# KKKSQJ/DeepLearning

Measured on NVIDIA H100. Metric: images/sec (ResNet-50 training step), higher is better.
Workload: dtype bf16

## Files before the change

deeplearning_b200/csrc/abi_conv.cu:

```cuda
#include <string.h>
#include "../../include/b200cls.h"
#include "conv_gemm.cuh"
#include "conv1x1_stream.cuh"
#include "conv_tap64.cuh"
#include "host_utils.h"
#include "wgrad_gemm.cuh"

using namespace b200;

namespace {

constexpr uint32_t kFwdDescLbo = 16, kFwdDescSbo = 1024;
constexpr uint32_t kWgDescLbo = 8192, kWgDescSbo = 1024, kWgDescKstep = 2048;

struct Box3 {
  int b1, b2, b3;
};

Box3 choose_box(long long d1, long long d2, long long d3, int P) {
  Box3 best{P, 1, 1};
  double best_cost = -1;
  for (int b1 = 1; b1 <= P; b1 <<= 1) {
    for (int b2 = 1; b1 * b2 <= P; b2 <<= 1) {
      const int b3 = P / (b1 * b2);
      if (b1 > 256 || b2 > 256 || b3 > 256) continue;
      const double c1 = double((d1 + b1 - 1) / b1) * b1, c2 = double((d2 + b2 - 1) / b2) * b2,
                   c3 = double((d3 + b3 - 1) / b3) * b3;
      const double cost = c1 * c2 * c3;
      if (best_cost < 0 || cost < best_cost - 0.5 ||
          (cost < best_cost + 0.5 && (b1 > best.b1 || (b1 == best.b1 && b2 > best.b2)))) {
        best_cost = cost;
        best = Box3{b1, b2, b3};
      }
    }
  }
  return best;
}

inline int pad_of(int ksize) { return ksize == 2 ? 0 : ksize / 2; }
inline int out_dim(int in, int ksize, int stride) { return (in + 2 * pad_of(ksize) - ksize) / stride + 1; }

struct Dims3 {
  long long d1, d2, d3;
};
Dims3 out_dims(int B, int H, int W, int ksize, int stride) {
  if (ksize == 1 && stride == 1) return Dims3{static_cast<long long>(B) * H * W, 1, 1};
  return Dims3{out_dim(W, ksize, stride), out_dim(H, ksize, stride), B};
}

struct View {
  const void* base;
  uint64_t dims[4];
  uint64_t strides[4];
};

View make_view(const void* base, int B, int H, int W, int C, int s, int ph, int pw) {
  View v;
  v.base = static_cast<const char*>(base) + (static_cast<long long>(ph) * W + pw) * C * 2;
  v.dims[0] = C;
  v.dims[1] = (W - pw + s - 1) / s;
  v.dims[2] = (H - ph + s - 1) / s;
  v.dims[3] = B;
  v.strides[0] = 1;
  v.strides[1] = static_cast<uint64_t>(s) * C;
  v.strides[2] = static_cast<uint64_t>(s) * W * C;
  v.strides[3] = static_cast<uint64_t>(H) * W * C;
  return v;
}
View make_flat_view(const void* base, long long M, int C) {
  View v;
  v.base = base;
  v.dims[0] = C;
  v.dims[1] = M;
  v.dims[2] = 1;
  v.dims[3] = 1;
  v.strides[0] = 1;
  v.strides[1] = C;
  v.strides[2] = static_cast<uint64_t>(M) * C;
  v.strides[3] = static_cast<uint64_t>(M) * C;
  return v;
}
View act_view(const void* base, int B, int H, int W, int C, bool flat) {
  return flat ? make_flat_view(base, static_cast<long long>(B) * H * W, C) : make_view(base, B, H, W, C, 1, 0, 0);
}
int encode_view(CUtensorMap* m, const View& v, const Box3& bx) {
  uint32_t box[4] = {64, (uint32_t)bx.b1, (uint32_t)bx.b2, (uint32_t)bx.b3};
  if (v.dims[1] == 0 || v.dims[2] == 0 || v.dims[3] == 0) {
// ... 34 lines not shown
  return OK;
}

void quarter_box(const Box3& bx, Box3* qb, int (&o1)[4], int (&o2)[4], int (&o3)[4]) {
  for (int q = 0; q < 4; ++q) o1[q] = o2[q] = o3[q] = 0;
  if (bx.b3 >= 4) {
    *qb = Box3{bx.b1, bx.b2, bx.b3 / 4};
    for (int q = 0; q < 4; ++q) o3[q] = q * (bx.b3 / 4);
  } else if (bx.b3 == 2) {
    *qb = Box3{bx.b1, bx.b2 / 2, 1};
    if (bx.b2 >= 2) {
      for (int q = 0; q < 4; ++q) {
        o2[q] = (q & 1) * (bx.b2 / 2);
        o3[q] = q >> 1;
      }
    } else {
      *qb = Box3{bx.b1 / 2, 1, 1};
      for (int q = 0; q < 4; ++q) {
        o1[q] = (q & 1) * (bx.b1 / 2);
        o3[q] = q >> 1;
      }
    }
  } else if (bx.b2 >= 4) {
    *qb = Box3{bx.b1, bx.b2 / 4, 1};
    for (int q = 0; q < 4; ++q) o2[q] = q * (bx.b2 / 4);
  } else if (bx.b2 == 2) {
    *qb = Box3{bx.b1 / 2, 1, 1};
    for (int q = 0; q < 4; ++q) {
      o1[q] = (q & 1) * (bx.b1 / 2);
      o2[q] = q >> 1;
    }
  } else {
    *qb = Box3{bx.b1 / 4, 1, 1};
    for (int q = 0; q < 4; ++q) o1[q] = q * (bx.b1 / 4);
  }
}

int setup_output(ConvGemmParams& p, const View& dv, int N, int out_f32, const View* auxv) {
  const long long d1 = dv.dims[1], d2 = dv.dims[2], d3 = dv.dims[3];
  const Box3 bx = choose_box(d1, d2, d3, 128);
  p.box1 = bx.b1, p.box2 = bx.b2, p.box3 = bx.b3;
  p.dim1 = static_cast<int>(d1), p.dim2 = static_cast<int>(d2), p.dim3 = static_cast<int>(d3);
  p.tiles1 = static_cast<int>((d1 + bx.b1 - 1) / bx.b1);
  p.tiles2 = static_cast<int>((d2 + bx.b2 - 1) / bx.b2);
  p.tiles3 = static_cast<int>((d3 + bx.b3 - 1) / bx.b3);
  p.N = N;
  const int BN = N <= 64 ? 64 : 128;
  p.n_tiles = (N + BN - 1) / BN;
  Box3 qb;
  quarter_box(bx, &qb, p.qoff1, p.qoff2, p.qoff3);
  p.out_f32 = out_f32;
  if (dv.base != nullptr) {
    uint32_t box[4] = {out_f32 ? 32u : 64u, (uint32_t)qb.b1, (uint32_t)qb.b2, (uint32_t)qb.b3};
    int rc = out_f32 ? encode_tmap_f32(&p.d_map, dv.base, 4, dv.dims, dv.strides, box)
                     : encode_tmap_bf16(&p.d_map, dv.base, 4, dv.dims, dv.strides, box);
    if (rc) return rc;
  }
  p.has_aux_out = 0;
  if (auxv != nullptr) {
    uint32_t box[4] = {64u, (uint32_t)qb.b1, (uint32_t)qb.b2, (uint32_t)qb.b3};
    int rc = encode_tmap_bf16(&p.aux_map, auxv->base, 4, auxv->dims, auxv->strides, box);
    if (rc) return rc;
    p.has_aux_out = 1;
  }
  return OK;
}
Box3 box_of(const ConvGemmParams& p) { return Box3{p.box1, p.box2, p.box3}; }

bool bn_mask_complete(const b200_bn_mask_t* m) { return m->x_raw && m->scale && m->shift && m->stats; }
void set_bn_mask(ConvGemmParams& p, const b200_bn_mask_t* m, const View& dv) {
  p.mask_in = static_cast<const __nv_bfloat16*>(m->x_raw);
  p.ms1 = static_cast<long long>(dv.strides[1]);
  p.ms2 = static_cast<long long>(dv.strides[2]);
  p.ms3 = static_cast<long long>(dv.strides[3]);
  p.bn_scale = m->scale, p.bn_shift = m->shift, p.stats = m->stats;
}

int conv_grid(int tiles, int n_tiles, bool stats) {
  int grid = tiles < device_sm_count() ? tiles : device_sm_count();
  if (stats) grid = grid / n_tiles * n_tiles;
  return grid;
}

template <int BLOCK_N, int EPI>
int launch_conv_gemm_epi(const ConvGemmParams& q, int grid, cudaStream_t st) {
  using Cfg = ConvGemmCfg<BLOCK_N>;
  static bool configured = false;
  if (!configured) {
    B200_CHECK_CUDA(cudaFuncSetAttribute(conv_gemm_kernel<BLOCK_N, EPI>, cudaFuncAttributeMaxDynamicSharedMemorySize,
                                         Cfg::SMEM_BYTES));
    configured = true;
  }
  B200_CHECK_CUDA(launch_pdl(conv_gemm_kernel<BLOCK_N, EPI>, dim3(grid), dim3(Cfg::THREADS), Cfg::SMEM_BYTES, st, q));
  B200_LAUNCHED();
  return OK;
}

int epilogue_flags(const ConvGemmParams& p) {
  int f = 0;
  if (p.bias) f |= kEpiBias;
  if (p.colscale) f |= kEpiColscale;
  f |= (p.act & 3) << kEpiActShift;
  if (p.residual) f |= p.res_f32 ? kEpiResF32 : kEpiResBf16;
  if (p.has_aux_out) f |= kEpiAux;
  if (p.out_f32) f |= kEpiOutF32;
  if (p.out_direct) f |= kEpiDirect;
  if (p.stats) f |= kEpiStats;
  if (p.rowscale) f |= kEpiRowscale;
  if (p.affine) f = (f & ~(kEpiBias | kEpiColscale)) | kEpiAffine;
  if (p.mask_in) f |= p.bn_scale ? kEpiBnMask : kEpiMask;
  if (p.bn_scale) f &= ~kEpiStats;
  return f;
}

#define B200_EPI_LIST(X)                                                                                  \
  X(kEpiStats)                                              \
  X(0)                                                      \
  X(kEpiResBf16)                                            \
  X(kEpiBias)                                               \
  X(kEpiBias | kEpiResF32 | kEpiOutF32)                     \
  X(kEpiBias | kEpiColscale | kEpiResF32 | kEpiOutF32)      \
  X(kEpiBias | (2 << kEpiActShift) | kEpiAux)               \
  X(3 << kEpiActShift)                                      \
  X((3 << kEpiActShift) | kEpiStats)                        \
  X(kEpiOutF32)                                             \
  X(kEpiBias | kEpiOutF32)                                  \
  X(kEpiAffine | kEpiResBf16 | (1 << kEpiActShift))        \
  X(kEpiAffine | (1 << kEpiActShift))                      \
  X(kEpiAffine)                                            \
  X(kEpiMask | kEpiResBf16 | kEpiStats)                    \
  X(kEpiBnMask)                                            \
  X(kEpiBnMask | kEpiBias)

bool tap64_ok(const ConvGemmParams& p) {
  const int f = epilogue_flags(p);
  return p.N == 64 && p.n_tiles == 1 && p.k_per_tap == 64 && p.k_blocks_per_tap == 1 && !p.var_taps && !p.chan_window &&
         p.num_taps >= 2 && p.num_taps <= 9 && (f == 0 || f == kEpiStats) && p.dim1 % p.box1 == 0 && p.dim2 % p.box2 == 0 &&
         p.dim3 % p.box3 == 0;
}
template <bool kStats>
int launch_tap64(const ConvGemmParams& q, int grid, cudaStream_t st) {
  static bool configured = false;
  if (!configured) {
    B200_CHECK_CUDA(cudaFuncSetAttribute(conv_tap64_kernel<kStats>, cudaFuncAttributeMaxDynamicSharedMemorySize, kTap64SmemBytes));
    configured = true;
  }
  B200_CHECK_CUDA(launch_pdl(conv_tap64_kernel<kStats>, dim3(grid), dim3(384), kTap64SmemBytes, st, q));
  B200_LAUNCHED();
  return OK;
}

template <int BLOCK_N>
int launch_conv_gemm(const ConvGemmParams& p, cudaStream_t st) {
  const int tiles = p.tiles1 * p.tiles2 * p.tiles3 * p.n_tiles;
  const int grid = conv_grid(tiles, p.n_tiles, p.stats != nullptr);
  B200_REQUIRE(grid > 0, "conv_gemm: %d channel blocks exceed the SM count (BN statistics need grid %% n_tiles == 0)", p.n_tiles);
  ConvGemmParams q = p;
  q.desc_lbo = kFwdDescLbo;
  q.desc_sbo = kFwdDescSbo;
  if constexpr (BLOCK_N == 64) {
    if (tap64_ok(p)) return p.stats != nullptr ? launch_tap64<true>(q, grid, st) : launch_tap64<false>(q, grid, st);
  }
  switch (epilogue_flags(p)) {
#define B200_EPI_CASE(F) \
  case (F):              \
    return launch_conv_gemm_epi<BLOCK_N, (F)>(q, grid, st);
    B200_EPI_LIST(B200_EPI_CASE)
#undef B200_EPI_CASE
    default:
      return launch_conv_gemm_epi<BLOCK_N, kEpiGeneric>(q, grid, st);
  }
}


bool stream_ok(long long pixels, int K, int N) {
  return (K == 64 || K == 128 || K == 256) && N % 256 == 0 && pixels % 128 == 0 && pixels / 128 < (1LL << 30);
}
int stream_grid(long long pixels, int N) {
  const int n_tiles = N / 256;
  const long long items = pixels / 128 * n_tiles;
  int grid = items < device_sm_count() ? static_cast<int>(items) : device_sm_count();
  return grid / n_tiles * n_tiles;
}

template <int KB, int MODE>
int launch_stream(const StreamParams& q, int grid, cudaStream_t st) {
  using Cfg = StreamCfg<KB, MODE>;
  static bool configured = false;
  if (!configured) {
    B200_CHECK_CUDA(cudaFuncSetAttribute(conv1x1_stream_kernel<KB, MODE>, cudaFuncAttributeMaxDynamicSharedMemorySize,
                                         Cfg::SMEM_BYTES));
    configured = true;
  }
  B200_CHECK_CUDA(launch_pdl(conv1x1_stream_kernel<KB, MODE>, dim3(grid), dim3(Cfg::THREADS), Cfg::SMEM_BYTES, st, q));
  B200_LAUNCHED();
  return OK;
}

int run_stream(int mode, const void* a, const void* w, void* out, const void* res, const void* mask, const float* scale,
               const float* shift, float* stats, long long pixels, int K, int N, cudaStream_t st) {
  StreamParams q;
  memset(&q, 0, sizeof(q));
  int rc;
  if ((rc = encode_matrix(&q.a_map, a, K, pixels, 128))) return rc;
  if ((rc = encode_matrix(&q.b_map, w, K, N, 256))) return rc;
  if ((rc = encode_matrix(&q.out_map, out, N, pixels, 16))) return rc;
  if (res != nullptr && (rc = encode_matrix(&q.res_map, res, N, pixels, 16))) return rc;
  if (mask != nullptr && (rc = encode_matrix(&q.mask_map, mask, N, pixels, 16))) return rc;
  q.m_tiles = static_cast<int>(pixels / 128);
  q.n_tiles = N / 256;
  q.N = N;
  q.scale = scale, q.shift = shift, q.stats = stats;
  const int grid = stream_grid(pixels, N);
  if (mode == kStreamAffine)
    return K == 64 ? launch_stream<1, kStreamAffine>(q, grid, st)
                   : (K == 128 ? launch_stream<2, kStreamAffine>(q, grid, st) : launch_stream<4, kStreamAffine>(q, grid, st));
  if (mode == kStreamBnRelu)
    return K == 64 ? launch_stream<1, kStreamBnRelu>(q, grid, st)
                   : (K == 128 ? launch_stream<2, kStreamBnRelu>(q, grid, st) : launch_stream<4, kStreamBnRelu>(q, grid, st));
  return K == 64 ? launch_stream<1, kStreamMask>(q, grid, st)
                 : (K == 128 ? launch_stream<2, kStreamMask>(q, grid, st) : launch_stream<4, kStreamMask>(q, grid, st));
}

int dispatch_conv_gemm(ConvGemmParams& p, int N, cudaStream_t st) {
  if (N <= 64) return launch_conv_gemm<64>(p, st);
  return launch_conv_gemm<128>(p, st);
}
int block_n_for(int N) { return N <= 64 ? 64 : 128; }

template <int BLOCK_NG, bool kGrouped = false>
int launch_wgrad(const WgradParams& p, cudaStream_t st) {
  using Cfg = WgradCfg<BLOCK_NG>;
  static bool configured = false;
  if (!configured) {
    if constexpr (kGrouped) {
      B200_CHECK_CUDA(cudaFuncSetAttribute(wgrad_gemm_kernel<BLOCK_NG, false, true>,
                                           cudaFuncAttributeMaxDynamicSharedMemorySize, Cfg::SMEM_BYTES));
    } else {
      B200_CHECK_CUDA(cudaFuncSetAttribute(wgrad_gemm_kernel<BLOCK_NG, false>, cudaFuncAttributeMaxDynamicSharedMemorySize,
                                           Cfg::SMEM_BYTES));
      B200_CHECK_CUDA(cudaFuncSetAttribute(wgrad_gemm_kernel<BLOCK_NG, true>, cudaFuncAttributeMaxDynamicSharedMemorySize,
                                           Cfg::SMEM_BYTES));
    }
    configured = true;
  }
  const int items = p.mg_tiles * p.ng_tiles * p.num_taps * p.splits;
// ... 594 lines not shown
```

deeplearning_b200/csrc/conv_gemm.cuh:

```cuda
#pragma once
#include <cstdio>
#include "common.cuh"

namespace b200 {

constexpr int kMaxTaps = 16;

struct alignas(64) ConvGemmParams {
  CUtensorMap a_maps[4];
  CUtensorMap b_map;
  CUtensorMap d_map;
  CUtensorMap aux_map;
  int num_taps;
  int k_per_tap;
  int k_blocks_per_tap;
  int tiles1, tiles2, tiles3;
  int box1, box2, box3;
  int dim1, dim2, dim3;
  int qoff1[4], qoff2[4], qoff3[4];
  int n_tiles;
  int N;
  int8_t tap_map[kMaxTaps];
  int8_t tap_o1[kMaxTaps];
  int8_t tap_o2[kMaxTaps];
  int8_t tap_w[kMaxTaps];
  float* stats;
  const float* bias;
  const float* colscale;
  int act;
  int out_f32;
  int res_f32;
  int has_aux_out;
  const void* residual;
  long long rs1, rs2, rs3;
  const __nv_bfloat16* aux_in;
  long long as1, as2, as3;
  uint32_t desc_lbo, desc_sbo;
  float* out_direct;
  long long ld_out;
  const float* rowscale;
  int rows_per_sample;
  int var_taps;
  int kb_total;
  int16_t tap_kb[kMaxTaps];
  int32_t tap_k0[kMaxTaps];
  const __nv_bfloat16* mask_in;
  long long ms1, ms2, ms3;
  int affine;
  const float* bn_scale;
  const float* bn_shift;
  int chan_window;
};

template <int BLOCK_N>
struct ConvGemmCfg {
  static constexpr int BLOCK_M = 128;
  static constexpr int BLOCK_K = 64;
  static constexpr int A_BYTES = BLOCK_M * BLOCK_K * 2;
  static constexpr int B_BYTES = BLOCK_N * BLOCK_K * 2;
  static constexpr int STAGES = BLOCK_N == 128 ? 4 : 5;
  static constexpr int STAGE_BYTES = A_BYTES + B_BYTES;
  static constexpr int EPI_WARPS = 4;
  static constexpr int SLAB_BYTES = 32 * 128;
  static constexpr int STAGING_BYTES = EPI_WARPS * 2 * SLAB_BYTES;
  static constexpr int IMG_BYTES = BLOCK_M * BLOCK_N * 4;
  static constexpr int IMGS = BLOCK_N == 128 ? 1 : 2;
  static constexpr int BAR_BYTES = 256;
  static constexpr int SMEM_BYTES = STAGES * STAGE_BYTES + STAGING_BYTES + IMGS * IMG_BYTES + BAR_BYTES + 1024;
  static constexpr int THREADS = 512;
  static_assert(SMEM_BYTES <= 227 * 1024, "shared memory of one H100 block");
  static_assert(2 * STAGES + 2 * IMGS <= BAR_BYTES / 8, "mbarriers");
};

__device__ __forceinline__ void gelu_parts(float x, float& tail, float& e) {
  const float az = fabsf(x) * 0.70710678118654752f;
  float t;
  asm("rcp.approx.ftz.f32 %0, %1;" : "=f"(t) : "f"(fmaf(0.3275911f, az, 1.0f)));
  float poly = fmaf(1.061405429f, t, -1.453152027f);
  poly = fmaf(poly, t, 1.421413741f);
  poly = fmaf(poly, t, -0.284496736f);
  poly = fmaf(poly, t, 0.254829592f);
  asm("ex2.approx.ftz.f32 %0, %1;" : "=f"(e) : "f"(-1.4426950408889634f * az * az));
  tail = 0.5f * poly * t * e;
}
__device__ __forceinline__ float gelu_erf(float x) {
  float tail, e;
  gelu_parts(x, tail, e);
  return x * (x >= 0.f ? 1.0f - tail : tail);
}
__device__ __forceinline__ float gelu_erf_grad(float x) {
  float tail, e;
  gelu_parts(x, tail, e);
  const float cdf = x >= 0.f ? 1.0f - tail : tail;
  return fmaf(x * 0.3989422804014327f, e, cdf);
}

__device__ __forceinline__ void gelu_parts2(float x0, float x1, uint64_t& cdf, uint64_t& e) {
  const uint64_t az = f2_pack(fabsf(x0) * 0.70710678118654752f, fabsf(x1) * 0.70710678118654752f);
  float d0, d1, t0, t1, g0, g1, e0, e1, h0, h1;
  f2_unpack(f2_fma(f2_bcast(0.3275911f), az, f2_bcast(1.0f)), d0, d1);
  asm("rcp.approx.ftz.f32 %0, %1;" : "=f"(t0) : "f"(d0));
  asm("rcp.approx.ftz.f32 %0, %1;" : "=f"(t1) : "f"(d1));
  const uint64_t t = f2_pack(t0, t1);
  uint64_t poly = f2_fma(f2_bcast(1.061405429f), t, f2_bcast(-1.453152027f));
  poly = f2_fma(poly, t, f2_bcast(1.421413741f));
  poly = f2_fma(poly, t, f2_bcast(-0.284496736f));
  poly = f2_fma(poly, t, f2_bcast(0.254829592f));
  f2_unpack(f2_mul(f2_mul(az, az), f2_bcast(-1.4426950408889634f)), g0, g1);
  asm("ex2.approx.ftz.f32 %0, %1;" : "=f"(e0) : "f"(g0));
  asm("ex2.approx.ftz.f32 %0, %1;" : "=f"(e1) : "f"(g1));
  e = f2_pack(e0, e1);
  f2_unpack(f2_fma(f2_mul(f2_mul(poly, t), e), f2_bcast(-0.5f), f2_bcast(0.5f)), h0, h1);
  cdf = f2_add(f2_pack(copysignf(h0, x0), copysignf(h1, x1)), f2_bcast(0.5f));
}
__device__ __forceinline__ void gelu_erf2(float& x0, float& x1) {
  uint64_t cdf, e;
  gelu_parts2(x0, x1, cdf, e);
  f2_unpack(f2_mul(f2_pack(x0, x1), cdf), x0, x1);
}
__device__ __forceinline__ void gelu_erf_val_grad2(float& x0, float& x1, float& g0, float& g1) {
  uint64_t cdf, e;
  gelu_parts2(x0, x1, cdf, e);
  const uint64_t x = f2_pack(x0, x1);
  f2_unpack(f2_fma(f2_mul(x, f2_bcast(0.3989422804014327f)), e, cdf), g0, g1);
  f2_unpack(f2_mul(x, cdf), x0, x1);
}

#ifdef CONV_PROFILE
#define CPROF_DECL(N) long long cp_t[N] = {}; long long cp_0 = clock64(), cp_1;
#define CPROF_TICK(i) { cp_1 = clock64(); cp_t[i] += cp_1 - cp_0; cp_0 = cp_1; }
#else
#define CPROF_DECL(N)
#define CPROF_TICK(i)
#endif

template <int S>
__device__ __forceinline__ void butterfly_step(float (&px)[32], int lane) {
  const bool up = (lane & S) != 0;
#pragma unroll
  for (int i = 0; i < S; ++i) {
    const float send = up ? px[i] : px[i + S];
    const float keep = up ? px[i + S] : px[i];
    px[i] = keep + __shfl_xor_sync(0xffffffffu, send, S);
  }
}

constexpr int kEpiGeneric = -1;
constexpr int kEpiBias = 1, kEpiColscale = 2, kEpiActShift = 2 , kEpiResBf16 = 16, kEpiResF32 = 32,
              kEpiAux = 64, kEpiOutF32 = 128, kEpiDirect = 256, kEpiStats = 512,
              kEpiRowscale = 1024 ,
              kEpiAffine = 2048, kEpiMask = 4096, kEpiBnMask = 8192;

template <int BLOCK_N, int EPI = kEpiGeneric>
__global__ void __launch_bounds__(512, 1) conv_gemm_kernel(const __grid_constant__ ConvGemmParams p) {
  static_assert(BLOCK_N == 64 || BLOCK_N == 128, "64- or 128-column tiles");
  using Cfg = ConvGemmCfg<BLOCK_N>;
  constexpr int STAGES = Cfg::STAGES;
  constexpr int IMGS = Cfg::IMGS;
  extern __shared__ uint8_t smem_raw[];
  uint8_t* smem = reinterpret_cast<uint8_t*>((reinterpret_cast<uintptr_t>(smem_raw) + 1023) & ~uintptr_t(1023));
  uint8_t* stage_base = smem;
  uint8_t* staging = smem + STAGES * Cfg::STAGE_BYTES;
  uint8_t* img = staging + Cfg::STAGING_BYTES;
  uint64_t* bars = reinterpret_cast<uint64_t*>(img + IMGS * Cfg::IMG_BYTES);
  uint64_t* full_bar = bars;
  uint64_t* empty_bar = bars + STAGES;
  uint64_t* img_full = bars + 2 * STAGES;
  uint64_t* img_empty = bars + 2 * STAGES + IMGS;

  const int warp_idx = threadIdx.x >> 5;
  const int lane = threadIdx.x & 31;
  const int m_tiles = p.tiles1 * p.tiles2 * p.tiles3;
  const int num_tiles = m_tiles * p.n_tiles;
  const int num_kb = p.var_taps ? p.kb_total : p.num_taps * p.k_blocks_per_tap;

  if (warp_idx == 0 && lane == 0) {
    for (int i = 0; i < 4; ++i) tma_prefetch_desc(&p.a_maps[i]);
    tma_prefetch_desc(&p.b_map);
    tma_prefetch_desc(&p.d_map);
    for (int i = 0; i < STAGES; ++i) {
      mbar_init(&full_bar[i], 1);
      mbar_init(&empty_bar[i], 2);
    }
    for (int i = 0; i < IMGS; ++i) {
      mbar_init(&img_full[i], 8);
      mbar_init(&img_empty[i], Cfg::EPI_WARPS);
    }
    fence_mbar_init();
  }
  __syncthreads();
  pdl_wait();

  if (warp_idx < 4) {
    setmaxnreg_dec<40>();
    if (warp_idx == 0 && lane == 0) {
      int stage = 0;
      uint32_t phase = 0;
      CPROF_DECL(2)
      for (int tile = blockIdx.x; tile < num_tiles; tile += gridDim.x) {
        const int n_tile = tile % p.n_tiles;
        const int m_tile = tile / p.n_tiles;
        const int t1 = m_tile % p.tiles1;
        const int t2 = (m_tile / p.tiles1) % p.tiles2;
        const int t3 = m_tile / (p.tiles1 * p.tiles2);
        const int c1 = t1 * p.box1, c2 = t2 * p.box2, c3 = t3 * p.box3;
        int tap = 0, cb = 0;
        int kb_in_tap = p.var_taps ? p.tap_kb[0] : p.k_blocks_per_tap;
        for (int kb = 0; kb < num_kb; ++kb, ++cb) {
          if (cb == kb_in_tap) {
            cb = 0;
            ++tap;
            if (p.var_taps) kb_in_tap = p.tap_kb[tap];
          }
          const int wk = p.var_taps ? p.tap_k0[tap] + cb * 64 : p.tap_w[tap] * p.k_per_tap + cb * 64;
          CPROF_TICK(1)
          mbar_wait_backoff(&empty_bar[stage], phase ^ 1);
          CPROF_TICK(0)
          uint8_t* a_dst = stage_base + stage * Cfg::STAGE_BYTES;
          uint8_t* b_dst = a_dst + Cfg::A_BYTES;
          mbar_expect_tx(&full_bar[stage], Cfg::STAGE_BYTES);
          tma_load_4d(a_dst, &p.a_maps[p.tap_map[tap]], &full_bar[stage], p.chan_window ? n_tile * BLOCK_N : cb * 64, c1 + p.tap_o1[tap],
                      c2 + p.tap_o2[tap], c3);
          tma_load_2d(b_dst, &p.b_map, &full_bar[stage], wk, n_tile * BLOCK_N);
          if (++stage == STAGES) {
            stage = 0;
            phase ^= 1;
          }
        }
      }
#ifdef CONV_PROFILE
      if (blockIdx.x == 0) {
        const int nt = (num_tiles - 1) / gridDim.x + 1;
        printf("conv producer: wait_empty %lld issue %lld  (cycles/tile, %d tiles, %d k-blocks)\n", cp_t[0] / nt, cp_t[1] / nt, nt, num_kb);
      }
#endif
    }
  } else if (warp_idx < 12) {
    setmaxnreg_dec<112>();
    const int wg = (warp_idx - 4) >> 2;
    const uint64_t desc_a0 = make_smem_desc_sw128(smem_u32(stage_base) + wg * 8192, p.desc_lbo, p.desc_sbo);
    const uint64_t desc_b0 = make_smem_desc_sw128(smem_u32(stage_base) + Cfg::A_BYTES, p.desc_lbo, p.desc_sbo);
    int stage = 0;
    uint32_t phase = 0;
    int it = 0;
    CPROF_DECL(3)
    for (int tile = blockIdx.x; tile < num_tiles; tile += gridDim.x, ++it) {
      float acc[BLOCK_N / 2];
#pragma unroll
      for (int i = 0; i < BLOCK_N / 2; ++i) acc[i] = 0.f;
      int prev = -1;
      CPROF_TICK(2)
      for (int kb = 0; kb < num_kb; ++kb) {
        mbar_wait(&full_bar[stage], phase);
        wgmma_fence();
        const uint64_t soff = static_cast<uint64_t>(stage) * (Cfg::STAGE_BYTES >> 4);
        const uint64_t da = desc_a0 + soff, db = desc_b0 + soff;
#pragma unroll
        for (int k = 0; k < 4; ++k) Wgmma<BLOCK_N, 0, 0>::mma(acc, da + 2 * k, db + 2 * k, 1u);
        wgmma_commit();
        wgmma_wait<1>();
        if (prev >= 0 && (threadIdx.x & 127) == 0) mbar_arrive(&empty_bar[prev]);
        prev = stage;
        if (++stage == STAGES) {
          stage = 0;
          phase ^= 1;
        }
      }
      wgmma_wait<0>();
      wgmma_reg_fence(acc);
      if ((threadIdx.x & 127) == 0) mbar_arrive(&empty_bar[prev]);
      CPROF_TICK(0)
      const int b = IMGS == 1 ? 0 : it % IMGS;
      mbar_wait(&img_empty[b], ((it / IMGS) & 1) ^ 1);
      CPROF_TICK(1)
      acc_to_img<BLOCK_N>(acc, smem_u32(img + b * Cfg::IMG_BYTES), BLOCK_N, 64 * wg, 0);
      __syncwarp();
      if (lane == 0) mbar_arrive(&img_full[b]);
    }
#ifdef CONV_PROFILE
    if (blockIdx.x == 0 && lane == 0 && (warp_idx & 3) == 0) {
      const int nt = (num_tiles - 1) / gridDim.x + 1;
      printf("conv mma wg %d: main loop %lld wait img_empty %lld acc->img %lld  (cycles/tile)\n", wg, cp_t[0] / nt, cp_t[1] / nt,
             cp_t[2] / nt);
    }
#endif
  } else {
    setmaxnreg_inc<248>();
    const int q = warp_idx - 12;
    const int row = q * 32 + lane;
    const uint32_t stage_s = smem_u32(staging + q * 2 * Cfg::SLAB_BYTES);
    const uint32_t row_s = lane * 128;
    const uint32_t sw = (lane & 7) << 4;
    uint32_t stat_off[8];
#pragma unroll
    for (int m = 0; m < 8; ++m) stat_off[m] = m * 128 + ((((lane >> 2) ^ m) << 4) | ((lane & 3) << 2));
    constexpr bool G = EPI < 0;
    constexpr bool kAffine = !G && (EPI & kEpiAffine) != 0;
    constexpr bool kBnMask = !G && (EPI & kEpiBnMask) != 0;
    constexpr bool kMask = !G && (EPI & (kEpiMask | kEpiBnMask)) != 0;
    const int N = p.N;
    const float* const bias = (!kAffine && (G || (EPI & kEpiBias))) ? p.bias : nullptr;
    const float* const colscale = (!kAffine && (G || (EPI & kEpiColscale))) ? p.colscale : nullptr;
    const int act_bits = G ? p.act : ((EPI >> kEpiActShift) & 3);
    const int act = kAffine ? 0 : act_bits;
    const bool has_res = G ? (p.residual != nullptr) : ((EPI & (kEpiResBf16 | kEpiResF32)) != 0);
    const bool res_f32 = G ? (p.res_f32 != 0) : ((EPI & kEpiResF32) != 0);
    const bool has_aux = G ? (p.has_aux_out != 0) : ((EPI & kEpiAux) != 0);
    const bool out_f32 = G ? (p.out_f32 != 0) : ((EPI & kEpiOutF32) != 0);
    float* const out_direct = (G || (EPI & kEpiDirect)) ? p.out_direct : nullptr;
    float* const stats = (G || (EPI & (kEpiStats | kEpiBnMask))) ? p.stats : nullptr;
    const float* const rowscale = G ? p.rowscale : nullptr;
    const bool need_rowmap = has_res || act == 3 || kMask || out_direct != nullptr || rowscale != nullptr || p.dim1 % p.box1 != 0 ||
                             p.dim2 % p.box2 != 0 || p.dim3 % p.box3 != 0;
    const bool full_cols = (N % BLOCK_N) == 0;
    uint32_t store_counter = 0;
    const int unit_cols = out_f32 ? 32 : 64;
    const int units = BLOCK_N / unit_cols;
    const int nsub = out_f32 ? 1 : 2;
    constexpr int SLOTS = 2;
    uint64_t run_s[SLOTS], run_q[SLOTS];
    float run_x[SLOTS][2];
#pragma unroll
    for (int k = 0; k < SLOTS; ++k) run_s[k] = 0, run_q[k] = 0, run_x[k][0] = run_x[k][1] = 0.f;
    int it = 0;
    CPROF_DECL(2)
    for (int tile = blockIdx.x; tile < num_tiles; tile += gridDim.x, ++it) {
      const int b = IMGS == 1 ? 0 : it % IMGS;
      const uint32_t img_s = smem_u32(img + b * Cfg::IMG_BYTES);
      const int n_tile = tile % p.n_tiles;
      const int m_tile = tile / p.n_tiles;
      const int t1 = m_tile % p.tiles1;
      const int t2 = (m_tile / p.tiles1) % p.tiles2;
      const int t3 = m_tile / (p.tiles1 * p.tiles2);
      const int c1 = t1 * p.box1, c2 = t2 * p.box2, c3 = t3 * p.box3;
      int p1 = 0, p2 = 0, p3 = 0;
      bool row_ok = true;
      if (need_rowmap) {
        const int i1 = row % p.box1;
        const int i2 = (row / p.box1) % p.box2;
        const int i3 = row / (p.box1 * p.box2);
        p1 = c1 + i1, p2 = c2 + i2, p3 = c3 + i3;
        row_ok = (p1 < p.dim1) && (p2 < p.dim2) && (p3 < p.dim3);
      }
      const int s1 = c1 + p.qoff1[q], s2 = c2 + p.qoff2[q], s3 = c3 + p.qoff3[q];

      uint4 nx_b[4];
      float4 nx_f[8];
      uint4 nx_m[4];
      auto issue_pre = [&](int u, int h) {
        const int ncp = n_tile * BLOCK_N + u * unit_cols + h * 32;
        if (n_tile * BLOCK_N + u * unit_cols >= N || !row_ok) return;
        if (has_res) {
          const long long off = p3 * p.rs3 + p2 * p.rs2 + p1 * p.rs1 + ncp;
          if (res_f32) {
            const float4* rp = reinterpret_cast<const float4*>(static_cast<const float*>(p.residual) + off);
#pragma unroll
            for (int j = 0; j < 8; ++j)
              if (full_cols || ncp + j * 4 < N) nx_f[j] = __ldg(rp + j);
          } else {
            const uint4* rp = reinterpret_cast<const uint4*>(static_cast<const __nv_bfloat16*>(p.residual) + off);
#pragma unroll
            for (int j = 0; j < 4; ++j)
              if (full_cols || ncp + j * 8 < N) nx_b[j] = __ldg(rp + j);
          }
        }
        if (act == 3) {
// ... 316 lines not shown
```

deeplearning_b200/csrc/conv_tap64.cuh:

```cuda
#pragma once
#include "conv_gemm.cuh"

namespace b200 {

constexpr int kTap64Stages = 5;
constexpr int kTap64SmemBytes = 9 * 8192 + kTap64Stages * 16384 + 8 * 4096 + 128 * 64 * 4 + 512 + 1024;
static_assert(kTap64SmemBytes <= 227 * 1024, "shared memory of one H100 block");

template <bool kStats>
__global__ void __launch_bounds__(384, 1) conv_tap64_kernel(const __grid_constant__ ConvGemmParams p) {
  constexpr int STAGES = kTap64Stages;
  extern __shared__ uint8_t smem_raw[];
  uint8_t* smem = reinterpret_cast<uint8_t*>((reinterpret_cast<uintptr_t>(smem_raw) + 1023) & ~uintptr_t(1023));
  uint8_t* sB = smem;
  uint8_t* sA = sB + 9 * 8192;
  uint8_t* sOut = sA + STAGES * 16384;
  uint8_t* sImg = sOut + 8 * 4096;
  uint64_t* bars = reinterpret_cast<uint64_t*>(sImg + 128 * 64 * 4);
  uint64_t* a_full = bars;
  uint64_t* a_empty = bars + STAGES;
  uint64_t* b_full = bars + 2 * STAGES;

  const int warp_idx = threadIdx.x >> 5, lane = threadIdx.x & 31;
  const int m_tiles = p.tiles1 * p.tiles2 * p.tiles3;
  const int taps = p.num_taps;

  if (warp_idx == 0 && lane == 0) {
    for (int i = 0; i < 4; ++i) tma_prefetch_desc(&p.a_maps[i]);
    tma_prefetch_desc(&p.b_map);
    tma_prefetch_desc(&p.d_map);
    for (int i = 0; i < STAGES; ++i) {
      mbar_init(&a_full[i], 1);
      mbar_init(&a_empty[i], 2);
    }
    mbar_init(b_full, 1);
    fence_mbar_init();
  }
  __syncthreads();
  pdl_wait();

  if (warp_idx < 4) {
    setmaxnreg_dec<40>();
    if (warp_idx == 0 && lane == 0) {
      mbar_expect_tx(b_full, static_cast<uint32_t>(taps) * 8192u);
      for (int t = 0; t < taps; ++t) tma_load_2d(sB + t * 8192, &p.b_map, b_full, p.tap_w[t] * p.k_per_tap, 0);
      int stage = 0;
      uint32_t phase = 0;
      for (int tile = blockIdx.x; tile < m_tiles; tile += gridDim.x) {
        const int t1 = tile % p.tiles1;
        const int t2 = (tile / p.tiles1) % p.tiles2;
        const int t3 = tile / (p.tiles1 * p.tiles2);
        const int c1 = t1 * p.box1, c2 = t2 * p.box2, c3 = t3 * p.box3;
        for (int t = 0; t < taps; ++t) {
          mbar_wait_backoff(&a_empty[stage], phase ^ 1);
          mbar_expect_tx(&a_full[stage], 16384);
          tma_load_4d(sA + stage * 16384, &p.a_maps[p.tap_map[t]], &a_full[stage], 0, c1 + p.tap_o1[t], c2 + p.tap_o2[t], c3);
          if (++stage == STAGES) {
            stage = 0;
            phase ^= 1;
          }
        }
      }
    }
  } else {
    setmaxnreg_inc<232>();
    const int ew = warp_idx - 4;
    const int wg = ew >> 2;
    const int q = 2 * wg + (ew & 1);
    const int pair = (ew >> 1) & 1;
    const int row = q * 32 + lane;
    const uint32_t img_s = smem_u32(sImg);
    const uint64_t desc_a0 = make_smem_desc_sw128(smem_u32(sA) + wg * 8192, p.desc_lbo, p.desc_sbo);
    const uint64_t desc_b0 = make_smem_desc_sw128(smem_u32(sB), p.desc_lbo, p.desc_sbo);
    const uint32_t os = smem_u32(sOut + ew * 4096);
    const uint32_t row_s = lane * 128;
    const uint32_t sw = (lane & 7) << 4;
    uint32_t stat_off[8];
#pragma unroll
    for (int m = 0; m < 8; ++m) stat_off[m] = m * 128 + ((((lane >> 2) ^ m) << 4) | ((lane & 3) << 2));
    uint64_t run_s = 0, run_q = 0;
    mbar_wait(b_full, 0);
    int stage = 0;
    uint32_t phase = 0;
    int it = 0;
    for (int tile = blockIdx.x; tile < m_tiles; tile += gridDim.x, ++it) {
      float acc[32];
#pragma unroll
      for (int i = 0; i < 32; ++i) acc[i] = 0.f;
      int prev = -1;
      for (int t = 0; t < taps; ++t) {
        mbar_wait(&a_full[stage], phase);
        wgmma_fence();
        const uint64_t da = desc_a0 + static_cast<uint64_t>(stage) * (16384 >> 4);
        const uint64_t db = desc_b0 + static_cast<uint64_t>(t) * (8192 >> 4);
#pragma unroll
        for (int k = 0; k < 4; ++k) Wgmma<64, 0, 0>::mma(acc, da + 2 * k, db + 2 * k, 1u);
        wgmma_commit();
        wgmma_wait<1>();
        if (prev >= 0 && (threadIdx.x & 127) == 0) mbar_arrive(&a_empty[prev]);
        prev = stage;
        if (++stage == STAGES) {
          stage = 0;
          phase ^= 1;
        }
      }
      wgmma_wait<0>();
      wgmma_reg_fence(acc);
      if ((threadIdx.x & 127) == 0) mbar_arrive(&a_empty[prev]);
      named_bar_sync(1 + wg, 128);
      acc_to_img<64>(acc, img_s, 64, 64 * wg, 0);
      named_bar_sync(1 + wg, 128);
      if ((it & 1) != pair) continue;
      const int t1 = tile % p.tiles1;
      const int t2 = (tile / p.tiles1) % p.tiles2;
      const int t3 = tile / (p.tiles1 * p.tiles2);
      const int s1 = t1 * p.box1 + p.qoff1[q], s2 = t2 * p.box2 + p.qoff2[q], s3 = t3 * p.box3 + p.qoff3[q];
      if (lane == 0) tma_store_wait_read<0>();
      __syncwarp();
#pragma unroll
      for (int h = 0; h < 2; ++h) {
        uint32_t v[32];
        img_ld32(img_s, 64, row, h * 32, v);
#pragma unroll
        for (int j = 0; j < 4; ++j)
          sts128(os + row_s + (((h * 4 + j) << 4) ^ sw),
                 pack_bf16x2(__uint_as_float(v[j * 8 + 0]), __uint_as_float(v[j * 8 + 1])),
                 pack_bf16x2(__uint_as_float(v[j * 8 + 2]), __uint_as_float(v[j * 8 + 3])),
                 pack_bf16x2(__uint_as_float(v[j * 8 + 4]), __uint_as_float(v[j * 8 + 5])),
                 pack_bf16x2(__uint_as_float(v[j * 8 + 6]), __uint_as_float(v[j * 8 + 7])));
      }
      __syncwarp();
      if constexpr (kStats) {
        uint64_t a_s = 0, a_q = 0;
#pragma unroll
        for (int r = 0; r < 32; ++r) {
          const uint32_t w = lds32(os + (r >> 3) * 1024 + stat_off[r & 7]);
          const uint64_t x2 = f2_pack(bf16_lo(w), bf16_hi(w));
          a_s = f2_add(a_s, x2);
          a_q = f2_fma(x2, x2, a_q);
        }
        run_s = f2_add(run_s, a_s);
        run_q = f2_add(run_q, a_q);
      }
      fence_proxy_async_smem();
      __syncwarp();
      if (lane == 0) {
        asm volatile("cp.async.bulk.tensor.4d.global.shared::cta.bulk_group [%0, {%2, %3, %4, %5}], [%1];" ::"l"(
                         reinterpret_cast<uint64_t>(&p.d_map)),
                     "r"(os), "r"(0), "r"(s1), "r"(s2), "r"(s3)
                     : "memory");
        tma_store_commit();
      }
    }
    if constexpr (kStats) {
      const long long srow = (static_cast<long long>(blockIdx.x) * 4 + q) * 2 + pair;
      float s_lo, s_hi, q_lo, q_hi;
      f2_unpack(run_s, s_lo, s_hi);
      f2_unpack(run_q, q_lo, q_hi);
      float* sp = p.stats + srow * 2 * p.N + 2 * lane;
      *reinterpret_cast<float2*>(sp) = make_float2(s_lo, s_hi);
      *reinterpret_cast<float2*>(sp + p.N) = make_float2(q_lo, q_hi);
    }
    if (lane == 0) tma_store_wait_all<0>();
  }
}

}
```

Baseline: 8784.

## Generalise resident-weight path into conv_gemm kernel and drop tap64 kernel

Replaces the specialised conv_tap64 kernel with a resident-B mode of the main conv_gemm kernel. When there is a single column tile and at most 9 K-blocks, the whole weight slab is loaded into shared memory once per block and only activations are streamed through the pipeline stages. This now covers more epilogues (BN mask, affine, generic) and variable-tap layouts, saving repeated weight TMA traffic per tile. In exchange, fewer pipeline stages fit in shared memory, and the former dedicated 384-thread stats epilogue is replaced by the generic 512-thread epilogue.

```diff
diff --git a/deeplearning_b200/csrc/abi_conv.cu b/deeplearning_b200/csrc/abi_conv.cu
--- a/deeplearning_b200/csrc/abi_conv.cu
+++ b/deeplearning_b200/csrc/abi_conv.cu
@@ -2,7 +2,6 @@
 #include "../../include/b200cls.h"
 #include "conv_gemm.cuh"
 #include "conv1x1_stream.cuh"
-#include "conv_tap64.cuh"
 #include "host_utils.h"
 #include "wgrad_gemm.cuh"
 
@@ -203,16 +202,16 @@
   return grid;
 }
 
-template <int BLOCK_N, int EPI>
+template <int BLOCK_N, int EPI, bool RES_B = false>
 int launch_conv_gemm_epi(const ConvGemmParams& q, int grid, cudaStream_t st) {
-  using Cfg = ConvGemmCfg<BLOCK_N>;
+  using Cfg = ConvGemmCfgOf<BLOCK_N, EPI, RES_B>;
   static bool configured = false;
   if (!configured) {
-    B200_CHECK_CUDA(cudaFuncSetAttribute(conv_gemm_kernel<BLOCK_N, EPI>, cudaFuncAttributeMaxDynamicSharedMemorySize,
+    B200_CHECK_CUDA(cudaFuncSetAttribute(conv_gemm_kernel<BLOCK_N, EPI, RES_B>, cudaFuncAttributeMaxDynamicSharedMemorySize,
                                          Cfg::SMEM_BYTES));
     configured = true;
   }
-  B200_CHECK_CUDA(launch_pdl(conv_gemm_kernel<BLOCK_N, EPI>, dim3(grid), dim3(Cfg::THREADS), Cfg::SMEM_BYTES, st, q));
+  B200_CHECK_CUDA(launch_pdl(conv_gemm_kernel<BLOCK_N, EPI, RES_B>, dim3(grid), dim3(Cfg::THREADS), Cfg::SMEM_BYTES, st, q));
   B200_LAUNCHED();
   return OK;
 }
@@ -253,22 +252,27 @@
   X(kEpiBnMask)                                            \
   X(kEpiBnMask | kEpiBias)
 
-bool tap64_ok(const ConvGemmParams& p) {
-  const int f = epilogue_flags(p);
-  return p.N == 64 && p.n_tiles == 1 && p.k_per_tap == 64 && p.k_blocks_per_tap == 1 && !p.var_taps && !p.chan_window &&
-         p.num_taps >= 2 && p.num_taps <= 9 && (f == 0 || f == kEpiStats) && p.dim1 % p.box1 == 0 && p.dim2 % p.box2 == 0 &&
-         p.dim3 % p.box3 == 0;
-}
-template <bool kStats>
-int launch_tap64(const ConvGemmParams& q, int grid, cudaStream_t st) {
-  static bool configured = false;
-  if (!configured) {
-    B200_CHECK_CUDA(cudaFuncSetAttribute(conv_tap64_kernel<kStats>, cudaFuncAttributeMaxDynamicSharedMemorySize, kTap64SmemBytes));
-    configured = true;
-  }
-  B200_CHECK_CUDA(launch_pdl(conv_tap64_kernel<kStats>, dim3(grid), dim3(384), kTap64SmemBytes, st, q));
-  B200_LAUNCHED();
-  return OK;
+#define B200_RESB_EPI_LIST(X)                                                                              \
+  X(kEpiStats)                                              \
+  X(kEpiBnMask)                                            \
+  X(kEpiBnMask | kEpiBias)                                 \
+  X(kEpiAffine | (1 << kEpiActShift))                      \
+  X(kEpiAffine)
+
+bool resident_b_ok(const ConvGemmParams& p) {
+  const int num_kb = p.var_taps ? p.kb_total : p.num_taps * p.k_blocks_per_tap;
+  return p.n_tiles == 1 && num_kb <= kResBMaxKb && !p.chan_window;
+}
+
+bool has_streamed_specialisation(int f) {
+  switch (f) {
+#define B200_EPI_CASE(F) case (F):
+    B200_EPI_LIST(B200_EPI_CASE)
+#undef B200_EPI_CASE
+    return true;
+    default:
+      return false;
+  }
 }
 
 template <int BLOCK_N>
@@ -279,10 +283,21 @@
   ConvGemmParams q = p;
   q.desc_lbo = kFwdDescLbo;
   q.desc_sbo = kFwdDescSbo;
+  const int f = epilogue_flags(p);
   if constexpr (BLOCK_N == 64) {
-    if (tap64_ok(p)) return p.stats != nullptr ? launch_tap64<true>(q, grid, st) : launch_tap64<false>(q, grid, st);
-  }
-  switch (epilogue_flags(p)) {
+    if (resident_b_ok(p)) {
+      switch (f) {
+#define B200_EPI_CASE(F) \
+  case (F):              \
+    return launch_conv_gemm_epi<64, (F), true>(q, grid, st);
+        B200_RESB_EPI_LIST(B200_EPI_CASE)
+#undef B200_EPI_CASE
+        default:
+          if (!has_streamed_specialisation(f)) return launch_conv_gemm_epi<64, kEpiGeneric, true>(q, grid, st);
+      }
+    }
+  }
+  switch (f) {
 #define B200_EPI_CASE(F) \
   case (F):              \
     return launch_conv_gemm_epi<BLOCK_N, (F)>(q, grid, st);
diff --git a/deeplearning_b200/csrc/conv_gemm.cuh b/deeplearning_b200/csrc/conv_gemm.cuh
--- a/deeplearning_b200/csrc/conv_gemm.cuh
+++ b/deeplearning_b200/csrc/conv_gemm.cuh
@@ -52,24 +52,29 @@
   int chan_window;
 };
 
-template <int BLOCK_N>
+constexpr int kResBMaxKb = 9;
+
+template <int BLOCK_N, int RES_IMGS = 0>
 struct ConvGemmCfg {
+  static constexpr bool RES_B = RES_IMGS > 0;
+  static_assert(!RES_B || BLOCK_N == 64, "resident weights: 64-column tiles only");
   static constexpr int BLOCK_M = 128;
   static constexpr int BLOCK_K = 64;
   static constexpr int A_BYTES = BLOCK_M * BLOCK_K * 2;
   static constexpr int B_BYTES = BLOCK_N * BLOCK_K * 2;
-  static constexpr int STAGES = BLOCK_N == 128 ? 4 : 5;
-  static constexpr int STAGE_BYTES = A_BYTES + B_BYTES;
+  static constexpr int B_RES_BYTES = RES_B ? kResBMaxKb * B_BYTES : 0;
+  static constexpr int STAGE_BYTES = RES_B ? A_BYTES : A_BYTES + B_BYTES;
   static constexpr int EPI_WARPS = 4;
   static constexpr int SLAB_BYTES = 32 * 128;
   static constexpr int STAGING_BYTES = EPI_WARPS * 2 * SLAB_BYTES;
   static constexpr int IMG_BYTES = BLOCK_M * BLOCK_N * 4;
-  static constexpr int IMGS = BLOCK_N == 128 ? 1 : 2;
+  static constexpr int IMGS = RES_B ? RES_IMGS : (BLOCK_N == 128 ? 1 : 2);
+  static constexpr int STAGES = RES_B ? (IMGS == 1 ? 5 : 3) : (BLOCK_N == 128 ? 4 : 5);
   static constexpr int BAR_BYTES = 256;
-  static constexpr int SMEM_BYTES = STAGES * STAGE_BYTES + STAGING_BYTES + IMGS * IMG_BYTES + BAR_BYTES + 1024;
+  static constexpr int SMEM_BYTES = B_RES_BYTES + STAGES * STAGE_BYTES + STAGING_BYTES + IMGS * IMG_BYTES + BAR_BYTES + 1024;
   static constexpr int THREADS = 512;
   static_assert(SMEM_BYTES <= 227 * 1024, "shared memory of one H100 block");
-  static_assert(2 * STAGES + 2 * IMGS <= BAR_BYTES / 8, "mbarriers");
+  static_assert(2 * STAGES + 2 * IMGS + 1 <= BAR_BYTES / 8, "mbarriers");
 };
 
 __device__ __forceinline__ void gelu_parts(float x, float& tail, float& e) {
@@ -151,22 +156,28 @@
               kEpiRowscale = 1024 ,
               kEpiAffine = 2048, kEpiMask = 4096, kEpiBnMask = 8192;
 
-template <int BLOCK_N, int EPI = kEpiGeneric>
+constexpr int resb_imgs(int epi) { return epi >= 0 && (epi & kEpiBnMask) == 0 ? 1 : 2; }
+template <int BLOCK_N, int EPI, bool RES_B>
+using ConvGemmCfgOf = ConvGemmCfg<BLOCK_N, RES_B ? resb_imgs(EPI) : 0>;
+
+template <int BLOCK_N, int EPI = kEpiGeneric, bool RES_B = false>
 __global__ void __launch_bounds__(512, 1) conv_gemm_kernel(const __grid_constant__ ConvGemmParams p) {
   static_assert(BLOCK_N == 64 || BLOCK_N == 128, "64- or 128-column tiles");
-  using Cfg = ConvGemmCfg<BLOCK_N>;
+  using Cfg = ConvGemmCfgOf<BLOCK_N, EPI, RES_B>;
   constexpr int STAGES = Cfg::STAGES;
   constexpr int IMGS = Cfg::IMGS;
   extern __shared__ uint8_t smem_raw[];
   uint8_t* smem = reinterpret_cast<uint8_t*>((reinterpret_cast<uintptr_t>(smem_raw) + 1023) & ~uintptr_t(1023));
-  uint8_t* stage_base = smem;
-  uint8_t* staging = smem + STAGES * Cfg::STAGE_BYTES;
+  uint8_t* b_res = smem;
+  uint8_t* stage_base = smem + Cfg::B_RES_BYTES;
+  uint8_t* staging = stage_base + STAGES * Cfg::STAGE_BYTES;
   uint8_t* img = staging + Cfg::STAGING_BYTES;
   uint64_t* bars = reinterpret_cast<uint64_t*>(img + IMGS * Cfg::IMG_BYTES);
   uint64_t* full_bar = bars;
   uint64_t* empty_bar = bars + STAGES;
   uint64_t* img_full = bars + 2 * STAGES;
   uint64_t* img_empty = bars + 2 * STAGES + IMGS;
+  uint64_t* b_full = bars + 2 * STAGES + 2 * IMGS;
 
   const int warp_idx = threadIdx.x >> 5;
   const int lane = threadIdx.x & 31;
@@ -186,6 +197,7 @@
       mbar_init(&img_full[i], 8);
       mbar_init(&img_empty[i], Cfg::EPI_WARPS);
     }
+    if (RES_B) mbar_init(b_full, 1);
     fence_mbar_init();
   }
   __syncthreads();
@@ -194,6 +206,22 @@
   if (warp_idx < 4) {
     setmaxnreg_dec<40>();
     if (warp_idx == 0 && lane == 0) {
+      auto for_each_kb = [&](auto&& body) {
+        int tap = 0, cb = 0;
+        int kb_in_tap = p.var_taps ? p.tap_kb[0] : p.k_blocks_per_tap;
+        for (int kb = 0; kb < num_kb; ++kb, ++cb) {
+          if (cb == kb_in_tap) {
+            cb = 0;
+            ++tap;
+            if (p.var_taps) kb_in_tap = p.tap_kb[tap];
+          }
+          body(kb, tap, cb, p.var_taps ? p.tap_k0[tap] + cb * 64 : p.tap_w[tap] * p.k_per_tap + cb * 64);
+        }
+      };
+      if constexpr (RES_B) {
+        mbar_expect_tx(b_full, static_cast<uint32_t>(num_kb) * Cfg::B_BYTES);
+        for_each_kb([&](int kb, int, int, int wk) { tma_load_2d(b_res + kb * Cfg::B_BYTES, &p.b_map, b_full, wk, 0); });
+      }
       int stage = 0;
       uint32_t phase = 0;
       CPROF_DECL(2)
@@ -204,29 +232,20 @@
         const int t2 = (m_tile / p.tiles1) % p.tiles2;
         const int t3 = m_tile / (p.tiles1 * p.tiles2);
         const int c1 = t1 * p.box1, c2 = t2 * p.box2, c3 = t3 * p.box3;
-        int tap = 0, cb = 0;
-        int kb_in_tap = p.var_taps ? p.tap_kb[0] : p.k_blocks_per_tap;
-        for (int kb = 0; kb < num_kb; ++kb, ++cb) {
-          if (cb == kb_in_tap) {
-            cb = 0;
-            ++tap;
-            if (p.var_taps) kb_in_tap = p.tap_kb[tap];
-          }
-          const int wk = p.var_taps ? p.tap_k0[tap] + cb * 64 : p.tap_w[tap] * p.k_per_tap + cb * 64;
+        for_each_kb([&](int, int tap, int cb, int wk) {
           CPROF_TICK(1)
           mbar_wait_backoff(&empty_bar[stage], phase ^ 1);
           CPROF_TICK(0)
           uint8_t* a_dst = stage_base + stage * Cfg::STAGE_BYTES;
-          uint8_t* b_dst = a_dst + Cfg::A_BYTES;
           mbar_expect_tx(&full_bar[stage], Cfg::STAGE_BYTES);
           tma_load_4d(a_dst, &p.a_maps[p.tap_map[tap]], &full_bar[stage], p.chan_window ? n_tile * BLOCK_N : cb * 64, c1 + p.tap_o1[tap],
                       c2 + p.tap_o2[tap], c3);
-          tma_load_2d(b_dst, &p.b_map, &full_bar[stage], wk, n_tile * BLOCK_N);
+          if constexpr (!RES_B) tma_load_2d(a_dst + Cfg::A_BYTES, &p.b_map, &full_bar[stage], wk, n_tile * BLOCK_N);
           if (++stage == STAGES) {
             stage = 0;
             phase ^= 1;
           }
-        }
+        });
       }
 #ifdef CONV_PROFILE
       if (blockIdx.x == 0) {
@@ -239,11 +258,15 @@
     setmaxnreg_dec<112>();
     const int wg = (warp_idx - 4) >> 2;
     const uint64_t desc_a0 = make_smem_desc_sw128(smem_u32(stage_base) + wg * 8192, p.desc_lbo, p.desc_sbo);
-    const uint64_t desc_b0 = make_smem_desc_sw128(smem_u32(stage_base) + Cfg::A_BYTES, p.desc_lbo, p.desc_sbo);
+    const uint64_t desc_b0 = make_smem_desc_sw128(RES_B ? smem_u32(b_res) : smem_u32(stage_base) + Cfg::A_BYTES, p.desc_lbo, p.desc_sbo);
     int stage = 0;
     uint32_t phase = 0;
     int it = 0;
-    CPROF_DECL(3)
+    CPROF_DECL(4)
+    if constexpr (RES_B) {
+      mbar_wait(b_full, 0);
+      CPROF_TICK(3)
+    }
     for (int tile = blockIdx.x; tile < num_tiles; tile += gridDim.x, ++it) {
       float acc[BLOCK_N / 2];
 #pragma unroll
@@ -254,7 +277,8 @@
         mbar_wait(&full_bar[stage], phase);
         wgmma_fence();
         const uint64_t soff = static_cast<uint64_t>(stage) * (Cfg::STAGE_BYTES >> 4);
-        const uint64_t da = desc_a0 + soff, db = desc_b0 + soff;
+        const uint64_t da = desc_a0 + soff;
+        const uint64_t db = desc_b0 + (RES_B ? static_cast<uint64_t>(kb) * (Cfg::B_BYTES >> 4) : soff);
 #pragma unroll
         for (int k = 0; k < 4; ++k) Wgmma<BLOCK_N, 0, 0>::mma(acc, da + 2 * k, db + 2 * k, 1u);
         wgmma_commit();
@@ -280,8 +304,8 @@
 #ifdef CONV_PROFILE
     if (blockIdx.x == 0 && lane == 0 && (warp_idx & 3) == 0) {
       const int nt = (num_tiles - 1) / gridDim.x + 1;
-      printf("conv mma wg %d: main loop %lld wait img_empty %lld acc->img %lld  (cycles/tile)\n", wg, cp_t[0] / nt, cp_t[1] / nt,
-             cp_t[2] / nt);
+      printf("conv mma wg %d: main loop %lld wait img_empty %lld acc->img %lld  (cycles/tile)  wait b_full %lld (cycles, once)\n", wg,
+             cp_t[0] / nt, cp_t[1] / nt, cp_t[2] / nt, cp_t[3]);
     }
 #endif
   } else {
diff --git a/deeplearning_b200/csrc/conv_tap64.cuh b/deeplearning_b200/csrc/conv_tap64.cuh
--- a/deeplearning_b200/csrc/conv_tap64.cuh
+++ /dev/null
@@ -1,168 +0,0 @@
-#pragma once
-#include "conv_gemm.cuh"
-
-namespace b200 {
-
-constexpr int kTap64Stages = 5;
-constexpr int kTap64SmemBytes = 9 * 8192 + kTap64Stages * 16384 + 8 * 4096 + 128 * 64 * 4 + 512 + 1024;
-static_assert(kTap64SmemBytes <= 227 * 1024, "shared memory of one H100 block");
-
-template <bool kStats>
-__global__ void __launch_bounds__(384, 1) conv_tap64_kernel(const __grid_constant__ ConvGemmParams p) {
-  constexpr int STAGES = kTap64Stages;
-  extern __shared__ uint8_t smem_raw[];
-  uint8_t* smem = reinterpret_cast<uint8_t*>((reinterpret_cast<uintptr_t>(smem_raw) + 1023) & ~uintptr_t(1023));
-  uint8_t* sB = smem;
-  uint8_t* sA = sB + 9 * 8192;
-  uint8_t* sOut = sA + STAGES * 16384;
-  uint8_t* sImg = sOut + 8 * 4096;
-  uint64_t* bars = reinterpret_cast<uint64_t*>(sImg + 128 * 64 * 4);
-  uint64_t* a_full = bars;
-  uint64_t* a_empty = bars + STAGES;
-  uint64_t* b_full = bars + 2 * STAGES;
-
-  const int warp_idx = threadIdx.x >> 5, lane = threadIdx.x & 31;
-  const int m_tiles = p.tiles1 * p.tiles2 * p.tiles3;
-  const int taps = p.num_taps;
-
-  if (warp_idx == 0 && lane == 0) {
-    for (int i = 0; i < 4; ++i) tma_prefetch_desc(&p.a_maps[i]);
-    tma_prefetch_desc(&p.b_map);
-    tma_prefetch_desc(&p.d_map);
-    for (int i = 0; i < STAGES; ++i) {
-      mbar_init(&a_full[i], 1);
-      mbar_init(&a_empty[i], 2);
-    }
-    mbar_init(b_full, 1);
-    fence_mbar_init();
-  }
-  __syncthreads();
-  pdl_wait();
-
-  if (warp_idx < 4) {
-    setmaxnreg_dec<40>();
-    if (warp_idx == 0 && lane == 0) {
-      mbar_expect_tx(b_full, static_cast<uint32_t>(taps) * 8192u);
-      for (int t = 0; t < taps; ++t) tma_load_2d(sB + t * 8192, &p.b_map, b_full, p.tap_w[t] * p.k_per_tap, 0);
-      int stage = 0;
-      uint32_t phase = 0;
-      for (int tile = blockIdx.x; tile < m_tiles; tile += gridDim.x) {
-        const int t1 = tile % p.tiles1;
-        const int t2 = (tile / p.tiles1) % p.tiles2;
-        const int t3 = tile / (p.tiles1 * p.tiles2);
-        const int c1 = t1 * p.box1, c2 = t2 * p.box2, c3 = t3 * p.box3;
-        for (int t = 0; t < taps; ++t) {
-          mbar_wait_backoff(&a_empty[stage], phase ^ 1);
-          mbar_expect_tx(&a_full[stage], 16384);
-          tma_load_4d(sA + stage * 16384, &p.a_maps[p.tap_map[t]], &a_full[stage], 0, c1 + p.tap_o1[t], c2 + p.tap_o2[t], c3);
-          if (++stage == STAGES) {
-            stage = 0;
-            phase ^= 1;
-          }
-        }
-      }
-    }
-  } else {
-    setmaxnreg_inc<232>();
-    const int ew = warp_idx - 4;
-    const int wg = ew >> 2;
-    const int q = 2 * wg + (ew & 1);
-    const int pair = (ew >> 1) & 1;
-    const int row = q * 32 + lane;
-    const uint32_t img_s = smem_u32(sImg);
-    const uint64_t desc_a0 = make_smem_desc_sw128(smem_u32(sA) + wg * 8192, p.desc_lbo, p.desc_sbo);
-    const uint64_t desc_b0 = make_smem_desc_sw128(smem_u32(sB), p.desc_lbo, p.desc_sbo);
-    const uint32_t os = smem_u32(sOut + ew * 4096);
-    const uint32_t row_s = lane * 128;
-    const uint32_t sw = (lane & 7) << 4;
-    uint32_t stat_off[8];
-#pragma unroll
-    for (int m = 0; m < 8; ++m) stat_off[m] = m * 128 + ((((lane >> 2) ^ m) << 4) | ((lane & 3) << 2));
-    uint64_t run_s = 0, run_q = 0;
-    mbar_wait(b_full, 0);
-    int stage = 0;
-    uint32_t phase = 0;
-    int it = 0;
-    for (int tile = blockIdx.x; tile < m_tiles; tile += gridDim.x, ++it) {
-      float acc[32];
-#pragma unroll
-      for (int i = 0; i < 32; ++i) acc[i] = 0.f;
-      int prev = -1;
-      for (int t = 0; t < taps; ++t) {
-        mbar_wait(&a_full[stage], phase);
-        wgmma_fence();
-        const uint64_t da = desc_a0 + static_cast<uint64_t>(stage) * (16384 >> 4);
-        const uint64_t db = desc_b0 + static_cast<uint64_t>(t) * (8192 >> 4);
-#pragma unroll
-        for (int k = 0; k < 4; ++k) Wgmma<64, 0, 0>::mma(acc, da + 2 * k, db + 2 * k, 1u);
-        wgmma_commit();
-        wgmma_wait<1>();
-        if (prev >= 0 && (threadIdx.x & 127) == 0) mbar_arrive(&a_empty[prev]);
-        prev = stage;
-        if (++stage == STAGES) {
-          stage = 0;
-          phase ^= 1;
-        }
-      }
-      wgmma_wait<0>();
-      wgmma_reg_fence(acc);
-      if ((threadIdx.x & 127) == 0) mbar_arrive(&a_empty[prev]);
-      named_bar_sync(1 + wg, 128);
-      acc_to_img<64>(acc, img_s, 64, 64 * wg, 0);
-      named_bar_sync(1 + wg, 128);
-      if ((it & 1) != pair) continue;
-      const int t1 = tile % p.tiles1;
-      const int t2 = (tile / p.tiles1) % p.tiles2;
-      const int t3 = tile / (p.tiles1 * p.tiles2);
-      const int s1 = t1 * p.box1 + p.qoff1[q], s2 = t2 * p.box2 + p.qoff2[q], s3 = t3 * p.box3 + p.qoff3[q];
-      if (lane == 0) tma_store_wait_read<0>();
-      __syncwarp();
-#pragma unroll
-      for (int h = 0; h < 2; ++h) {
-        uint32_t v[32];
-        img_ld32(img_s, 64, row, h * 32, v);
-#pragma unroll
-        for (int j = 0; j < 4; ++j)
-          sts128(os + row_s + (((h * 4 + j) << 4) ^ sw),
-                 pack_bf16x2(__uint_as_float(v[j * 8 + 0]), __uint_as_float(v[j * 8 + 1])),
-                 pack_bf16x2(__uint_as_float(v[j * 8 + 2]), __uint_as_float(v[j * 8 + 3])),
-                 pack_bf16x2(__uint_as_float(v[j * 8 + 4]), __uint_as_float(v[j * 8 + 5])),
-                 pack_bf16x2(__uint_as_float(v[j * 8 + 6]), __uint_as_float(v[j * 8 + 7])));
-      }
-      __syncwarp();
-      if constexpr (kStats) {
-        uint64_t a_s = 0, a_q = 0;
-#pragma unroll
-        for (int r = 0; r < 32; ++r) {
-          const uint32_t w = lds32(os + (r >> 3) * 1024 + stat_off[r & 7]);
-          const uint64_t x2 = f2_pack(bf16_lo(w), bf16_hi(w));
-          a_s = f2_add(a_s, x2);
-          a_q = f2_fma(x2, x2, a_q);
-        }
-        run_s = f2_add(run_s, a_s);
-        run_q = f2_add(run_q, a_q);
-      }
-      fence_proxy_async_smem();
-      __syncwarp();
-      if (lane == 0) {
-        asm volatile("cp.async.bulk.tensor.4d.global.shared::cta.bulk_group [%0, {%2, %3, %4, %5}], [%1];" ::"l"(
-                         reinterpret_cast<uint64_t>(&p.d_map)),
-                     "r"(os), "r"(0), "r"(s1), "r"(s2), "r"(s3)
-                     : "memory");
-        tma_store_commit();
-      }
-    }
-    if constexpr (kStats) {
-      const long long srow = (static_cast<long long>(blockIdx.x) * 4 + q) * 2 + pair;
-      float s_lo, s_hi, q_lo, q_hi;
-      f2_unpack(run_s, s_lo, s_hi);
-      f2_unpack(run_q, q_lo, q_hi);
-      float* sp = p.stats + srow * 2 * p.N + 2 * lane;
-      *reinterpret_cast<float2*>(sp) = make_float2(s_lo, s_hi);
-      *reinterpret_cast<float2*>(sp + p.N) = make_float2(q_lo, q_hi);
-    }
-    if (lane == 0) tma_store_wait_all<0>();
-  }
-}
-
-}
```

Result: no change. 8856, median of 6 (+0.8%).
